# WeltXing/PyDyNet

Hardware: AMD Instinct MI355X
Metric: training-step samples/sec (6L Llama3, seq=256) (higher is better)
Workload: dtype f32

## Files before the change

pydynet_amd/csrc/common.h:

```cpp
#pragma once
#include <hip/hip_runtime.h>
#include <stdint.h>
#include <stdio.h>
#include <string.h>

#define PDN_MAX_DIMS 8

enum {
  PDN_OK = 0,
  PDN_EINVAL = -1,
  PDN_EUNSUPPORTED = -2,
  PDN_EWORKSPACE = -3,
};

void pdn_set_error(const char* fmt, ...);

enum {
  PDN_CNT_ROWRES_CHUNK = 0,
  PDN_CNT_ROWTILE_PLAIN = 1,
  PDN_CNT_ROWTILE_SWIGLU_FWD = 2,
  PDN_CNT_ROWTILE_SWIGLU_BWD = 3,
  PDN_CNT_ROWTILE_ROPE = 4,
  PDN_CNT_ROWTILE_ROWMAX = 5,
  PDN_CNT_ROWRES_CHUNK_EPI = 6,
  PDN_CNT_ATT_P_FWD = 7,
  PDN_CNT_ATT_P_BWD = 8,
  PDN_CNT_ATT_RES_FWD = 9,
  PDN_CNT_ATT_RES_BWD = 10,
  PDN_CNT_ATT_STREAM = 11,
  PDN_CNT_CE_DX_DEFERRED = 12,
  PDN_CNT_CE_DW = 13,
  PDN_CNT_OUTRES = 14,
  PDN_CNT_OUTRES_TN = 15,
  PDN_CNT_LINEAR_RELU_FWD = 16,
  PDN_CNT_LINEAR_DX_MASKED = 17,
  PDN_CNT_CE_SMALL = 18,
  PDN_CNT_TILED_SWIGLU_FWD = 19,
  PDN_CNT_TILED_SWIGLU_BWD = 20,
  PDN_CNT_CONV_QUAD_FWD = 21,
  PDN_CNT_CONV_QUAD_DGRAD = 22,
  PDN_CNT_CONV_QUAD_WGRAD = 23,
  PDN_CNT_PATCH_EMBED_FWD = 24,
  PDN_CNT_PATCH_EMBED_BWD = 25,
  PDN_CNT_L2NORM_FWD = 26,
  PDN_CNT_L2NORM_BWD = 27,
  PDN_CNT_SAMPLE = 28,
  PDN_CNT_DECODE_ROWS = 29,
  PDN_CNT_DECODE_SLOTS = 30,
  PDN_CNT_DECODE_WIDE = 31,
  PDN_CNT_BEAM = 32,
  PDN_CNT_EXTEND = 33,
  PDN_CNT_SPECULATE = 34,
  PDN_CNT_PENALTY = 35,
  PDN_CNT_LOGPROBS = 36,
  PDN_CNT_LMHEAD_SPLIT = 37,
  PDN_CNT_PREFIX = 38,
  PDN_CNT_CE_DX_SPLIT = 39,
  PDN_CNT_CE_DW_SPLIT = 40,
  PDN_CNT_ROWTILE_SPLIT = 41,
  PDN_CNT_OUTRES_TN_SPLIT = 42,
  PDN_CNT_ATT_SEG = 43,
  PDN_CNT_ROW_LOSS = 44,
  PDN_CNT_SMOOTH_LOSS = 45,
  PDN_CNT_OUTRES_SPLIT = 46,
  PDN_CNT_SLOTS = 47
};
void pdn_count(int slot);

#define PDN_CHECK_ARG(cond, ...)          \
  do {                                    \
    if (!(cond)) {                        \
      pdn_set_error(__VA_ARGS__);         \
      return PDN_EINVAL;                  \
    }                                     \
  } while (0)

#define PDN_LAUNCH_CHECK()                                            \
  do {                                                                \
    hipError_t _e = hipGetLastError();                                \
    if (_e != hipSuccess) {                                           \
      pdn_set_error("%s:%d launch failed: %s", __FILE__, __LINE__,    \
                    hipGetErrorString(_e));                           \
      return (int)_e;                                                 \
    }                                                                 \
  } while (0)

#define PDN_HIP(call)                                                 \
  do {                                                                \
    hipError_t _e = (call);                                           \
    if (_e != hipSuccess) {                                           \
      pdn_set_error("%s:%d %s: %s", __FILE__, __LINE__, #call,        \
                    hipGetErrorString(_e));                           \
      return (int)_e;                                                 \
    }                                                                 \
  } while (0)

static inline int64_t cdiv64(int64_t a, int64_t b) { return (a + b - 1) / b; }

struct PdnView {
  int ndim;
  int64_t shape[PDN_MAX_DIMS];
  int64_t stride[PDN_MAX_DIMS];
};

__device__ __forceinline__ float wave_sum(float v) {
#pragma unroll
  for (int o = 32; o > 0; o >>= 1) v += __shfl_xor(v, o, 64);
  return v;
}
__device__ __forceinline__ float wave_max(float v) {
#pragma unroll
  for (int o = 32; o > 0; o >>= 1) v = fmaxf(v, __shfl_xor(v, o, 64));
  return v;
}
__device__ __forceinline__ double wave_sum(double v) {
#pragma unroll
  for (int o = 32; o > 0; o >>= 1) v += __shfl_xor(v, o, 64);
  return v;
// ... 53 lines not shown
```

pydynet_amd/csrc/gemm.hip:

```cpp
#include "common.h"
#include <vector>
#include <mutex>
#include <stdlib.h>
#include <stdio.h>
#include <type_traits>

#include "gemm_tiled.h"
#include "gemm_stream.h"
#include "split_tn.h"

struct TileCfg {
  int waves_m, waves_n, wm, wn, bk;
  float eff;
};
static const TileCfg kCfgs[] = {
    {2, 2, 2, 2, 32, 1.00f},
    {4, 1, 1, 3, 32, 0.97f},
    {1, 4, 3, 1, 32, 0.95f},
    {4, 1, 1, 2, 32, 0.85f},
    {1, 4, 2, 1, 32, 0.90f},
    {2, 2, 1, 1, 32, 0.60f},
    {2, 2, 4, 2, 16, 0.85f},
    {2, 2, 2, 4, 16, 1.10f},
    {4, 1, 2, 3, 16, 0.99f},
// ... 72 lines not shown
#define PDN_GEMM_FAMILIES 5
extern "C" int pdn_gemm_prof_collect_families(double* ms5, double* flops5, int64_t* launches5) {
  std::lock_guard<std::mutex> lk(g_prof_mu);
  double ms[PDN_GEMM_FAMILIES] = {0}, fl[PDN_GEMM_FAMILIES] = {0};
  int64_t n[PDN_GEMM_FAMILIES] = {0};
  for (auto& r : g_prof) {
    PDN_HIP(hipEventSynchronize(r.e1));
    float t = 0.f;
    PDN_HIP(hipEventElapsedTime(&t, r.e0, r.e1));
    const int f = r.family == 5 ? 2 : (r.family < 0 || r.family >= PDN_GEMM_FAMILIES ? 0 : r.family);
    ms[f] += t; fl[f] += r.flops; n[f]++;
    (void)hipEventDestroy(r.e0);
    (void)hipEventDestroy(r.e1);
  }
  for (int f = 0; f < PDN_GEMM_FAMILIES; ++f) {
    if (ms5) ms5[f] = ms[f];
    if (flops5) flops5[f] = fl[f];
    if (launches5) launches5[f] = n[f];
  }
  g_prof.clear();
  return PDN_OK;
}

extern "C" int pdn_gemm_prof_collect(double* total_ms, double* total_flops, int64_t* launches) {
  double ms[PDN_GEMM_FAMILIES], fl[PDN_GEMM_FAMILIES];
  int64_t n[PDN_GEMM_FAMILIES];
  int rc = pdn_gemm_prof_collect_families(ms, fl, n);
  if (rc) return rc;
  double tm = 0, tf = 0;
  int64_t tn = 0;
  for (int f = 0; f < PDN_GEMM_FAMILIES; ++f) { tm += ms[f]; tf += fl[f]; tn += n[f]; }
  if (total_ms) *total_ms = tm;
  if (total_flops) *total_flops = tf;
  if (launches) *launches = tn;
  return PDN_OK;
}

int pdn_gemm_outres_tn_plan(int N, int K, int* nw_out, int* k_per_split_out);
int pdn_gemm_outres_tn_launch(const float* X, const float* G, float* C, int N, int K, int64_t ldx, int64_t ldg,
                              int64_t ldc, int64_t slab, int nw, int k_per_split, void* stream);
int pdn_gemm_outres_tn_blocks_launch(const float* X, const float* G, float* C, int N, int K, int64_t ldx, int64_t ldg,
                                     int nb_cols, int nw, int k_per_split, void* stream);
extern "C" int64_t pdn_gemm_outres_workspace_bytes(int M, int K);
extern "C" int pdn_gemm_outres_plan(int M, int K, int* nw, int* kps);
extern "C" int pdn_gemm_outres_ws_f32(const float* A, const float* B, float* C, const float* bias, const float* residual,
                                      int M, int N, int K, int64_t lda, int64_t ldb, int64_t ldc, int b_trans,
                                      void* workspace, int64_t workspace_bytes, void* stream);
extern "C" int pdn_gemm_outres_supported(int M, int N, int K, int64_t lda, int64_t ldb, int64_t ldc, int b_trans);
extern "C" int pdn_gemm_outres_f32(const float* A, const float* B, float* C, const float* bias,
                                   const float* residual, int M, int N, int K, int64_t lda, int64_t ldb,
                                   int64_t ldc, int b_trans, void* stream);
extern "C" int pdn_gemm_rowres_supported(int M, int N, int K, int64_t lda, int64_t ldb, int64_t ldc, int b_trans);
int pdn_rowtile_plain_ok(int M, int N, int b_trans);
extern "C" int pdn_gemm_rowres_f32(const float* A, const float* B, float* C, const float* bias,
                                   const float* residual, int M, int N, int K, int64_t lda, int64_t ldb,
                                   int64_t ldc, int b_trans, void* stream);
int pdn_gemm_rowres_blocks(const float* A, const float* B, float* C, int M, int N, int K, int64_t lda, int64_t ldb,
                           int64_t ldc, int b_trans, int nblocks, int64_t b_block_stride, void* stream);

extern "C" int64_t pdn_gemm_f32_workspace_bytes(int M, int N, int K, int nbatch) {
  const int64_t base = (int64_t)64 * M * N * (int64_t)nbatch * 4;
  if (!pdn_outres_tn_split_supported(M, N, nbatch, K)) return base;
  return ((base + 255) & ~(int64_t)255) + pdn_outres_tn_split_extra_bytes(K);
}

bool pdn_gemm_narrow_nn_ok(int M, int N, int K, int64_t a_rs, int64_t a_cs, const void* A);
int pdn_gemm_narrow_nn_launch(const float* A, int64_t lda, const float* B, int64_t b_rs, int64_t b_cs, const float* bias,
                              float* C, int64_t ldc, int M, int N, int K, void* stream);
int pdn_gemm_narrow_tn_plan(int Mc, int N, int K, int64_t a_rs, int64_t a_cs, int64_t b_cs, const void* A, int64_t ws_cap_floats,
                            int* kps);
int pdn_gemm_narrow_tn_launch(const float* A, int64_t a_cs, const float* B, int64_t b_rs, float* slabs, int Mc, int N, int K,
                              int kps, int splits, void* stream);

static int gemm_f32_impl(int M, int N, int K, float alpha, const float* A, int64_t a_rs,
                         int64_t a_cs, const float* B, int64_t b_rs, int64_t b_cs, float beta,
                         float* C, int64_t ldc, const float* bias, int nb1, int nb2,
                         int64_t a_bs1, int64_t a_bs2, int64_t b_bs1, int64_t b_bs2,
                         int64_t c_bs1, int64_t c_bs2, const float* residual,
                         float* b_colsum, int colsum_accumulate, void* workspace,
                         int64_t workspace_bytes, void* stream, uint32_t* relu_mask, const uint32_t* grad_mask,
                         float* mask_colsum = nullptr) {
  const bool ext_on = relu_mask || grad_mask;
  PDN_CHECK_ARG(!ext_on || (nb1 == 1 && nb2 == 1 && N % 32 == 0 && !b_colsum),
                "pdn_gemm_f32: the mask epilogues need one batch and N a multiple of 32 (N = %d)", N);
  PDN_CHECK_ARG(M >= 0 && N >= 0 && K >= 0 && nb1 >= 0 && nb2 >= 0, "pdn_gemm_f32: negative extent");
  if (M == 0 || N == 0 || nb1 == 0 || nb2 == 0) return PDN_OK;
  PDN_CHECK_ARG(A && B && C, "pdn_gemm_f32: null operand");
  PDN_CHECK_ARG(ldc >= N, "pdn_gemm_f32: ldc (%lld) < N (%d)", (long long)ldc, N);
  hipStream_t st = (hipStream_t)stream;
  const int nbatch = nb1 * nb2;

  GemmParams p;
  p.A = A; p.B = B; p.C = C; p.bias = bias; p.ws = (float*)workspace;
  p.residual = residual; p.colsum = b_colsum; p.colsum_acc = colsum_accumulate;
  p.relu_mask = relu_mask; p.grad_mask = grad_mask; p.mask_colsum = grad_mask ? mask_colsum : nullptr;
  p.M = M; p.N = N; p.K = K;
  p.a_rs = a_rs; p.a_cs = a_cs; p.b_rs = b_rs; p.b_cs = b_cs; p.ldc = ldc;
  p.nb2 = nb2;
  p.a_bs1 = a_bs1; p.a_bs2 = a_bs2; p.b_bs1 = b_bs1; p.b_bs2 = b_bs2; p.c_bs1 = c_bs1; p.c_bs2 = c_bs2;
  p.alpha = alpha; p.beta = beta;

  const bool a_kin = !(a_rs == 1 && a_cs != 1) || M == 1;
  const bool b_kin = (b_rs == 1 && b_cs != 1) || (b_rs == 1 && N == 1);
  auto al16 = [](const void* q) { return ((uintptr_t)q & 15) == 0; };
  auto m4 = [](int64_t v) { return (v & 3) == 0; };
  bool vec = al16(A) && al16(B) && m4(a_bs1) && m4(a_bs2) && m4(b_bs1) && m4(b_bs2);
// ... 26 lines not shown
      if (getenv("PDN_GEMM_DEBUG")) fprintf(stderr, "pdn_gemm_f32 M=%d N=%d K=%d -> narrow NN\n", M, N, K);
      return pdn_gemm_narrow_nn_launch(A, a_rs, B, b_rs, b_cs, bias, C, ldc, M, N, K, stream);
    }
    int kps = 0;
    const int64_t cap = (workspace && workspace_bytes > 0 && al16(workspace)) ? workspace_bytes / 4 : 0;
    const int sp = !bias ? pdn_gemm_narrow_tn_plan(M, N, K, a_rs, a_cs, b_cs, A, cap, &kps) : 0;
    if (sp > 0) {
      if (getenv("PDN_GEMM_DEBUG")) fprintf(stderr, "pdn_gemm_f32 M=%d N=%d K=%d -> narrow TN (%d slabs)\n", M, N, K, sp);
      const int rc = pdn_gemm_narrow_tn_launch(A, a_cs, B, b_rs, (float*)workspace, M, N, K, kps, sp, stream);
      if (rc) return rc;
      p.splits = sp;
      const int64_t total = (int64_t)M * N;
      const int blocks = (int)((total + 255) / 256 < 2048 ? (total + 255) / 256 : 2048);
      const int rvec = (N % 4 == 0) && (ldc % 4 == 0) && al16(C);
      hipLaunchKernelGGL(gemm_splitk_reduce_kernel, dim3(blocks), dim3(256), 0, st, p, 1, rvec);
      PDN_LAUNCH_CHECK();
      return PDN_OK;
    }
  }
  if (nbatch == 1 && !ext_on && N == 288 && a_cs == 1 && alpha == 1.f && beta == 0.f && !b_colsum && K >= 768 &&
      al16(A) && al16(B) && !getenv("PDN_GEMM_NO_OUTRES")) {
    const int bt = (b_rs == 1 && b_cs != 1) ? 1 : 0;
    const int64_t ldb = bt ? b_cs : b_rs;
    const bool big = (M + 255) / 256 >= 224, mid = (M + 127) / 128 >= 224 && K >= 1536;
    int pl_nw, pl_kps;
    const int64_t or_ws = (workspace && workspace_bytes > 0) ? workspace_bytes : 0;
    const bool cut = !big && M >= 8192 && K >= 1536 && pdn_gemm_outres_plan(M, K, &pl_nw, &pl_kps) > 1 &&
                     or_ws >= pdn_gemm_outres_workspace_bytes(M, K);
    if ((big || mid || cut) && (bt || b_cs == 1) && pdn_gemm_outres_supported(M, N, K, a_rs, ldb, ldc, bt)) {
      bool prof;
      ProfRec rec;
      {
        std::lock_guard<std::mutex> lk(g_prof_mu);
        prof = g_prof_on;
      }
      if (prof) {
        PDN_HIP(hipEventCreate(&rec.e0));
        PDN_HIP(hipEventCreate(&rec.e1));
        rec.flops = 2.0 * M * (double)N * (double)K;
        rec.family = 3;
        PDN_HIP(hipEventRecord(rec.e0, st));
      }
      if (getenv("PDN_GEMM_DEBUG"))
        fprintf(stderr, "pdn_gemm_f32 M=%d N=%d K=%d -> output-resident (%s)\n", M, N, K, bt ? "NT" : "NN");
      const int rc = cut ? pdn_gemm_outres_ws_f32(A, B, C, bias, residual, M, N, K, a_rs, ldb, ldc, bt, workspace, or_ws, stream)
                         : pdn_gemm_outres_f32(A, B, C, bias, residual, M, N, K, a_rs, ldb, ldc, bt, stream);
      if (rc) return rc;
      if (prof) {
        PDN_HIP(hipEventRecord(rec.e1, st));
        std::lock_guard<std::mutex> lk(g_prof_mu);
        g_prof.push_back(rec);
      }
      return PDN_OK;
    }
  }
  {
    const bool one_dim = nb1 == 1 || nb2 == 1;
    const int64_t a_bs = nb1 == 1 ? a_bs2 : a_bs1, b_bs = nb1 == 1 ? b_bs2 : b_bs1, c_bs = nb1 == 1 ? c_bs2 : c_bs1;
    const bool blocks = nbatch > 1 && one_dim && a_bs == 0 && c_bs == N && ldc >= (int64_t)nbatch * N && !bias &&
                        N % 96 == 0 && (b_bs & 3) == 0;
    const int64_t n_all = (int64_t)N * (blocks ? nbatch : 1);
    const int bt0 = (b_rs == 1 && b_cs != 1) ? 1 : 0;
    const bool tilepiece = nbatch == 1 && K == 288 && n_all >= 96 && n_all % 32 == 0 && M >= 8192 &&
                           pdn_rowtile_plain_ok(M, (int)n_all, bt0);
    if ((nbatch == 1 || blocks) && !ext_on && K == 288 && a_cs == 1 && alpha == 1.f && beta == 0.f && !b_colsum &&
        (tilepiece || (!residual && n_all >= 768)) && n_all < (1 << 30) && M >= 8192 && al16(A) && al16(B) &&
        (!residual || al16(residual)) && !getenv("PDN_GEMM_NO_ROWRES")) {
      const int bt = (b_rs == 1 && b_cs != 1) ? 1 : 0;
      const int64_t ldb = bt ? b_cs : b_rs;
      if ((bt || b_cs == 1) && pdn_gemm_rowres_supported(M, N, K, a_rs, ldb, ldc, bt)) {
        bool prof;
        ProfRec rec;
        {
          std::lock_guard<std::mutex> lk(g_prof_mu);
          prof = g_prof_on;
        }
        if (prof) {
          PDN_HIP(hipEventCreate(&rec.e0));
          PDN_HIP(hipEventCreate(&rec.e1));
          rec.flops = 2.0 * M * (double)n_all * (double)K;
          rec.family = 2;
          PDN_HIP(hipEventRecord(rec.e0, st));
        }
        if (getenv("PDN_GEMM_DEBUG"))
          fprintf(stderr, "pdn_gemm_f32 M=%d N=%lld K=%d -> row-resident (%s, %d block%s)\n", M, (long long)n_all, K,
                  bt ? "NT" : "NN", blocks ? nbatch : 1, blocks ? "s" : "");
        const int rc = blocks ? pdn_gemm_rowres_blocks(A, B, C, M, (int)n_all, K, a_rs, ldb, ldc, bt, nbatch, b_bs, stream)
                              : pdn_gemm_rowres_f32(A, B, C, bias, residual, M, N, K, a_rs, ldb, ldc, bt, stream);
        if (rc) return rc;
        if (prof) {
          PDN_HIP(hipEventRecord(rec.e1, st));
          std::lock_guard<std::mutex> lk(g_prof_mu);
          g_prof.push_back(rec);
        }
        return PDN_OK;
      }
    }
  }
  const int64_t ws_cap = (workspace && workspace_bytes > 0) ? workspace_bytes / 4 : 0;
  if (nbatch == 1 && !ext_on && M == 288 && a_rs == 1 && a_cs >= 288 && b_cs == 1 && alpha == 1.f && !b_colsum && !bias && !residual &&
      N >= 8192 && N % 32 == 0 && K % 32 == 0 && K >= 4096 && m4(a_cs) && m4(b_rs) && al16(A) && al16(B) &&
      (int64_t)288 * ldc < (1ll << 30) && (int64_t)32 * b_rs < (1ll << 30) && !getenv("PDN_GEMM_NO_OUTRES")) {
    int nw = 8, kps = K;
    const int splits = pdn_gemm_outres_tn_plan(N, K, &nw, &kps);
    const bool direct = splits == 1 && beta == 0.f;
    if (direct || (int64_t)splits * M * N <= ws_cap) {
// ... 562 lines not shown
```

pydynet_amd/csrc/gemm_outres.hip:

```cpp
#include "common.h"
#include <stdlib.h>

static int pdn_ablation_switch(const char* name) {
  const char* e = getenv(name);
  const int v = e ? atoi(e) : 0;
  if (v) fprintf(stderr, "[pdnhip] WARNING: %s=%d -- timing ablation active, results of the affected kernels are WRONG\n", name, v);
  return v;
}

typedef float f32x16 __attribute__((ext_vector_type(16)));

struct OutResParams {
  const float* A;
  const float* B;
  float* C;
  const float* bias;
  const float* residual;
  int M, K;
  int64_t lda, ldb, ldc;
  const float* lse;
  const int64_t* targets;
  const float* gdev;
  float gscale;
  int kps;
// ... 346 lines not shown
  int nw, kps;
  const int splits = pdn_gemm_outres_plan(M, K, &nw, &kps);
  return splits > 1 ? (int64_t)splits * M * OR_N * 4 : 0;
}

extern "C" int pdn_gemm_outres_supported(int M, int N, int K, int64_t lda, int64_t ldb, int64_t ldc, int b_trans) {
  return N == OR_N && K >= OR_KP && K % OR_KP == 0 && M >= 1 && lda % 4 == 0 && ldb % 4 == 0 && lda >= K &&
         ldb >= (b_trans ? K : N) && ldc >= N && (int64_t)OR_N * ldb < (1ll << 30) && (int64_t)32 * ldc < (1ll << 30);
}

static int outres_launch(const float* A, const float* B, float* C, const float* bias, const float* residual, int M, int N,
                         int K, int64_t lda, int64_t ldb, int64_t ldc, int b_trans, void* workspace,
                         int64_t workspace_bytes, void* stream, int kb = 0, int64_t b_bstride = 0);

extern "C" int pdn_gemm_outres_f32(const float* A, const float* B, float* C, const float* bias,
                                   const float* residual, int M, int N, int K, int64_t lda, int64_t ldb,
                                   int64_t ldc, int b_trans, void* stream) {
  return outres_launch(A, B, C, bias, residual, M, N, K, lda, ldb, ldc, b_trans, nullptr, 0, stream);
}

extern "C" int pdn_gemm_outres_ws_f32(const float* A, const float* B, float* C, const float* bias,
                                      const float* residual, int M, int N, int K, int64_t lda, int64_t ldb,
                                      int64_t ldc, int b_trans, void* workspace, int64_t workspace_bytes, void* stream) {
  return outres_launch(A, B, C, bias, residual, M, N, K, lda, ldb, ldc, b_trans, workspace, workspace_bytes, stream);
}

int pdn_gemm_prof_begin(int family, double flops, double bytes, void* stream);
void pdn_gemm_prof_end(int token, void* stream);

extern "C" int pdn_gemm_outres_blocks_supported(int M, int kb, int nb) {
  const int K = kb * nb;
  const bool big = (M + 255) / 256 >= 224, mid = (M + 127) / 128 >= 224 && K >= 1536;
  return (kb > 0 && kb % OR_KP == 0 && nb >= 1 && (big || mid)) ? 1 : 0;
}
extern "C" int pdn_gemm_outres_blocks_nt_f32(const float* A, const float* W, int64_t b_block_stride, int kb, int nb, float* C,
                                             const float* residual, int M, int64_t lda, int64_t ldc, void* stream) {
  if (M == 0) return PDN_OK;
  const int K = kb * nb;
  if (!pdn_gemm_outres_blocks_supported(M, kb, nb) || (b_block_stride & 3) || (kb & 3) ||
      !pdn_gemm_outres_supported(M, OR_N, K, lda, K, ldc, 1)) {
    pdn_set_error("pdn_gemm_outres_blocks_nt_f32: unsupported shape M=%d kb=%d nb=%d", M, kb, nb);
    return PDN_EUNSUPPORTED;
  }
  const int tk = pdn_gemm_prof_begin(3, 2.0 * M * (double)OR_N * K, 0.0, stream);
  const int rc = outres_launch(A, W, C, nullptr, residual, M, OR_N, K, lda, kb, ldc, 1, nullptr, 0, stream, kb, b_block_stride);
  pdn_gemm_prof_end(tk, stream);
  return rc;
}

int pdn_outres_split_takes(const float* A, const float* B, const float* C, const float* bias, const float* residual, int M,
                           int K, int64_t lda, int64_t ldb, int64_t ldc, int b_trans, int kb, int64_t b_bstride, int splits,
                           void* stream);
int pdn_outres_split_launch(const float* A, const float* B, float* C, const float* bias, const float* residual, int M, int K,
                            int64_t lda, int64_t ldb, int64_t ldc, int b_trans, int kb, int64_t b_bstride, void* stream);

static int outres_launch(const float* A, const float* B, float* C, const float* bias, const float* residual, int M, int N,
                         int K, int64_t lda, int64_t ldb, int64_t ldc, int b_trans, void* workspace,
                         int64_t workspace_bytes, void* stream, int kb, int64_t b_bstride) {
  if (M == 0 || N == 0) return PDN_OK;
  PDN_CHECK_ARG(A && B && C, "pdn_gemm_outres_f32: null operand");
  if (!pdn_gemm_outres_supported(M, N, K, lda, kb > 0 ? K : ldb, ldc, b_trans)) {
    pdn_set_error("pdn_gemm_outres_f32: unsupported shape M=%d N=%d K=%d (N 288, K a multiple of 32, leading "
                  "dimensions multiples of 4)", M, N, K);
    return PDN_EUNSUPPORTED;
  }
  PDN_CHECK_ARG(((((uintptr_t)A | (uintptr_t)B) & 15) == 0), "pdn_gemm_outres_f32: 16-byte alignment required");
  OutResParams p{A, B, C, bias, residual, M, K, lda, ldb, ldc, nullptr, nullptr, nullptr, 0.f, K / OR_KP, nullptr};
  static const int s_pdn_outres_rt_ablate = pdn_ablation_switch("PDN_OUTRES_RT_ABLATE");
  p.ablate_rt = s_pdn_outres_rt_ablate;
  if (kb > 0) {
    p.ppb = kb / OR_KP;
    p.ppb_magic = (unsigned)(((1ull << 32) + (unsigned)p.ppb - 1) / (unsigned)p.ppb);
    p.b_bstride = b_bstride;
  }
  hipStream_t st = (hipStream_t)stream;
  int plan_nw = 8, kps = K / OR_KP;
  int splits = pdn_gemm_outres_plan(M, K, &plan_nw, &kps);
  if (splits > 1 && (!workspace || workspace_bytes < (int64_t)splits * M * OR_N * 4 || (ldc & 3) ||
                     ((uintptr_t)C & 15) || ((uintptr_t)workspace & 15) || ((uintptr_t)bias & 15) || ((uintptr_t)residual & 15))) {
    splits = 1;
    plan_nw = outres_unsplit_nw(M);
  }
  if (splits > 1) { p.kps = kps; p.slab = (float*)workspace; }
  if (pdn_outres_split_takes(A, B, C, bias, residual, M, K, lda, ldb, ldc, b_trans, kb, b_bstride, splits, stream)) {
    const int rc = pdn_outres_split_launch(A, B, C, bias, residual, M, K, lda, ldb, ldc, b_trans, kb, b_bstride, stream);
    if (rc == PDN_OK) pdn_count(PDN_CNT_OUTRES);
    return rc;
  }
  static const int nw_env = getenv("PDN_OUTRES_NW") ? atoi(getenv("PDN_OUTRES_NW")) : 0;
  static const int stage_env = getenv("PDN_OUTRES_STAGE") ? atoi(getenv("PDN_OUTRES_STAGE")) : -1;
  static const int ablate = pdn_ablation_switch("PDN_OUTRES_ABLATE");
  const int nw = nw_env ? nw_env : plan_nw;
  const int stage = stage_env >= 0 ? stage_env : 1;
  const dim3 grid((M + 32 * nw - 1) / (32 * nw), splits);
  pdn_count(PDN_CNT_OUTRES);
#define OR_LAUNCH(BT_, NW_, ST_, AB_) hipLaunchKernelGGL((gemm_outres_kernel<BT_, NW_, ST_, AB_>), grid, dim3(NW_ * 64), 0, st, p)
  if (ablate == 1 && b_trans) OR_LAUNCH(true, 4, 1, 1);
  else if (ablate == 2 && b_trans) OR_LAUNCH(true, 4, 1, 2);
  else if (nw == 8 && b_trans) { if (stage) OR_LAUNCH(true, 8, 1, 0); else OR_LAUNCH(true, 8, 0, 0); }
  else if (nw == 8) { if (stage) OR_LAUNCH(false, 8, 1, 0); else OR_LAUNCH(false, 8, 0, 0); }
  else if (b_trans) { if (stage) OR_LAUNCH(true, 4, 1, 0); else OR_LAUNCH(true, 4, 0, 0); }
  else { if (stage) OR_LAUNCH(false, 4, 1, 0); else OR_LAUNCH(false, 4, 0, 0); }
#undef OR_LAUNCH
  PDN_LAUNCH_CHECK();
  if (splits > 1) {
    const int64_t n4 = (int64_t)M * (OR_N / 4);
    hipLaunchKernelGGL(outres_splitk_reduce_kernel, dim3((unsigned)((n4 + 255) / 256)), dim3(256), 0, st, p.slab, splits, M,
                       bias, residual, C, ldc);
    PDN_LAUNCH_CHECK();
  }
  return PDN_OK;
}

int pdn_outres_ce_dx_launch(const float* logits, int64_t ldl, const float* lse, const int64_t* targets, float gscale,
                            const float* gdev, const float* W, int64_t ldw, float* dx, int64_t ldc,
                            const float* residual, int M, int V, void* workspace, int64_t workspace_bytes, void* stream) {
  OutResParams p{logits, W, dx, nullptr, residual, M, V, ldl, ldw, ldc, lse, targets, gdev, gscale, V / OR_KP, nullptr};
  int nw = 8, kps = V / OR_KP;
  int splits = pdn_gemm_outres_plan(M, V, &nw, &kps);
  if (splits > 1 && (!workspace || workspace_bytes < (int64_t)splits * M * OR_N * 4 || (ldc & 3) || ((uintptr_t)dx & 15) ||
                     ((uintptr_t)workspace & 15) || ((uintptr_t)residual & 15))) {
    splits = 1;
    nw = outres_unsplit_nw(M);
  }
  if (splits > 1) { p.kps = kps; p.slab = (float*)workspace; }
  const dim3 grid((M + 32 * nw - 1) / (32 * nw), splits);
  if (nw == 8) hipLaunchKernelGGL((gemm_outres_kernel<true, 8, 1, 0, 1>), grid, dim3(512), 0, (hipStream_t)stream, p);
  else hipLaunchKernelGGL((gemm_outres_kernel<true, 4, 1, 0, 1>), grid, dim3(256), 0, (hipStream_t)stream, p);
  PDN_LAUNCH_CHECK();
  if (splits > 1) {
    const int64_t n4 = (int64_t)M * (OR_N / 4);
    hipLaunchKernelGGL(outres_splitk_reduce_kernel, dim3((unsigned)((n4 + 255) / 256)), dim3(256), 0, (hipStream_t)stream,
                       p.slab, splits, M, (const float*)nullptr, residual, dx, ldc);
    PDN_LAUNCH_CHECK();
  }
  return PDN_OK;
}

// ... 409 lines not shown
```

pydynet_amd/csrc/outres_split.hip:

```cpp
#include "split_tn.h"
#include "outres_split_index.h"

extern "C" int pdn_malloc(void** ptr, int64_t bytes);
extern "C" int pdn_free(void* ptr);

struct OrsWParams {
  const float* B;
  float* pmax;
  int* wsh;
  char* wimg;
  int np, ppb;
  int64_t ldb, bstride;
};

__device__ __forceinline__ float ors_finite_or_inf(float a) { return a < INFINITY ? a : INFINITY; }

template <bool NN>
__device__ __forceinline__ void ors_w_unit(const OrsWParams& p, const float* tile, int d, int q, float (&v)[8]) {
  if (NN) {
#pragma unroll
    for (int j = 0; j < 8; ++j) v[j] = tile[ors_nn_lds(8 * q + j, d)];
  } else {
    const float* src = p.B + ors_w_src_nt(blockIdx.x, d, q, p.ppb, p.ldb, p.bstride);
    const float4 a = *reinterpret_cast<const float4*>(src);
    const float4 b = *reinterpret_cast<const float4*>(src + 4);
    v[0] = a.x; v[1] = a.y; v[2] = a.z; v[3] = a.w; v[4] = b.x; v[5] = b.y; v[6] = b.z; v[7] = b.w;
  }
}
__device__ __forceinline__ void ors_w_stage_nn(const OrsWParams& p, float* tile) {
  for (int i = threadIdx.x; i < ORS_KP * (ORS_N / 4); i += 256) {
    const float4 a = *reinterpret_cast<const float4*>(p.B + ors_w_src_nn(blockIdx.x, i, p.ldb));
    float* t = tile + ors_nn_lds(i / 72, 4 * (i % 72));
    t[0] = a.x; t[1] = a.y; t[2] = a.z; t[3] = a.w;
  }
  __syncthreads();
}

template <bool NN>
__global__ __launch_bounds__(256) void ors_w_max_kernel(OrsWParams p) {
  __shared__ float tile[NN ? ORS_KP * ORS_NN_LD : 1];
  if (NN) ors_w_stage_nn(p, tile);
  for (int i = threadIdx.x; i < ORS_N * 4; i += 256) {
    const int d = i >> 2, q = i & 3;
    float v[8];
    ors_w_unit<NN>(p, tile, d, q, v);
    float m = 0.f;
#pragma unroll
    for (int j = 0; j < 8; ++j) m = fmaxf(m, ors_finite_or_inf(fabsf(v[j])));
    m = fmaxf(m, __shfl_xor(m, 1, 64));
    m = fmaxf(m, __shfl_xor(m, 2, 64));
    if (q == 0) p.pmax[(int64_t)blockIdx.x * ORS_N + d] = m;
  }
}

template <bool NN>
__global__ __launch_bounds__(256) void ors_w_img_kernel(OrsWParams p) {
  __shared__ float tile[NN ? ORS_KP * ORS_NN_LD : 1];
  if (NN) ors_w_stage_nn(p, tile);
  char* img = p.wimg + (int64_t)blockIdx.x * ORS_PIECE;
  for (int i = threadIdx.x; i < ORS_N * 4; i += 256) {
    const int d = i >> 2, q = i & 3;
    float amax = 0.f;
    for (int s = 0; s < p.np; ++s) amax = fmaxf(amax, p.pmax[(int64_t)s * ORS_N + d]);
    const int sh = ls_shift(amax);
    if (blockIdx.x == 0 && q == 0) p.wsh[d] = sh;
    float v[8];
    ors_w_unit<NN>(p, tile, d, q, v);
    f16x8 hv, lv;
#pragma unroll
    for (int j = 0; j < 8; ++j) {
      _Float16 h, l;
      ls_split(v[j], sh, h, l);
      hv[j] = h; lv[j] = l;
    }
    char* dst = img + ors_img_unit(d, q);
    *reinterpret_cast<f16x8*>(dst) = hv;
    *reinterpret_cast<f16x8*>(dst + ORS_PLANE) = lv;
  }
}

struct OrsParams {
  const float* A;
  const char* wimg;
  const int* wsh;
  const float* bias;
  const float* residual;
  float* C;
  int M, np, nblk;
  int64_t lda, ldc;
};

__device__ __forceinline__ float ors_max8(const float4& a, const float4& b) {
  const float v[8] = {a.x, a.y, a.z, a.w, b.x, b.y, b.z, b.w};
  float m = 0.f;
#pragma unroll
  for (int j = 0; j < 8; ++j) {
    const float f = fabsf(v[j]);
    m = fmaxf(m, f < INFINITY ? f : 0.f);
  }
  return m;
}
__device__ __forceinline__ int ors_step_exp(float mx, int S) { return ors_next_exp(mx > 0.f, __builtin_amdgcn_frexp_expf(mx), S); }
__device__ __forceinline__ void ors_form2(float x0, float x1, int S, unsigned& hp, unsigned& lp) {
  f16x2 h, l;
  _Float16 a, b;
  ls_split_scaled(ldexpf(x0, S), a, b);
  h[0] = a; l[0] = b;
  ls_split_scaled(ldexpf(x1, S), a, b);
  h[1] = a; l[1] = b;
  hp = __builtin_bit_cast(unsigned, h);
  lp = __builtin_bit_cast(unsigned, l);
  asm volatile("" : "+v"(hp), "+v"(lp));
}

template <int ABLATE>
__global__ __launch_bounds__(512, 1) void ors_main_kernel(OrsParams p) {
  __shared__ __attribute__((aligned(1024))) char smem[ORS_LDS];
  const int tid = threadIdx.x, lane = tid & 63;
  const int wave = __builtin_amdgcn_readfirstlane(tid >> 6);
  const int r = lane & 15, q = lane >> 4;
  const int np = p.np, nblk = p.nblk, grid = gridDim.x;
  const unsigned lds0 = (unsigned)(size_t)(__attribute__((address_space(3))) char*)smem;
  constexpr bool STREAM = ABLATE == 0 || ABLATE == 3;

  const char* wsrc = p.wimg + lane * 16;
  auto dma_w = [&](int piece, int slot) __attribute__((always_inline)) {
    const char* src = wsrc + (int64_t)piece * ORS_PIECE;
#pragma unroll
    for (int e = 0; e < 5; ++e) {
      const int I = ors_wdma_instr(e, wave);
      split_dma16(src + I * 1024, __builtin_amdgcn_readfirstlane(lds0 + slot + I * 1024));
    }
  };
  auto a_src = [&](int blk, int i) __attribute__((always_inline)) {
    return p.A + ors_a_row(blk, wave, ors_raw_row(i, lane), p.M) * p.lda + 4 * ors_raw_chunk(i, lane);
  };
  int blk = blockIdx.x, nxt = ors_next_block(blk, grid, nblk);
  const float* ac0 = a_src(blk, 0);
  const float* ac1 = a_src(blk, 1);
  const float* an0 = a_src(nxt, 0);
  const float* an1 = a_src(nxt, 1);
  const int rw_base = ORS_RING0 + wave * (ORS_RING * ORS_RAW);
  auto dma_raw = [&](const float* s0, const float* s1, int piece, int ring) __attribute__((always_inline)) {
    const int64_t o = (int64_t)piece * ORS_KP;
    split_dma16(s0 + o, __builtin_amdgcn_readfirstlane(lds0 + rw_base + ring * ORS_RAW));
    split_dma16(s1 + o, __builtin_amdgcn_readfirstlane(lds0 + rw_base + ring * ORS_RAW + 1024));
  };
  const int raw_lane = rw_base + ors_raw_lane(r, q);

  dma_w(0, 0);
  if (ABLATE != 1) { dma_raw(ac0, ac1, 0, 0); dma_raw(ac0, ac1, 1, 1); dma_raw(ac0, ac1, 2, 2); dma_raw(ac0, ac1, 3, 3); }
  asm volatile("s_waitcnt vmcnt(0)" ::: "memory");
  f16x8 bh, bl;
#pragma unroll
  for (int j = 0; j < 8; ++j) { bh[j] = (_Float16)1.f; bl[j] = (_Float16)0.5f; }
  int S = ABLATE == 1 ? 0 : ORS_UNSET;
  if (ABLATE != 1) {
    const float4 v0 = *reinterpret_cast<const float4*>(__builtin_assume_aligned(smem + raw_lane, 16));
    const float4 v1 = *reinterpret_cast<const float4*>(__builtin_assume_aligned(smem + (raw_lane ^ 16), 16));
    float mx = ors_max8(v0, v1);
    mx = fmaxf(mx, __shfl_xor(mx, 16, 64));
    mx = fmaxf(mx, __shfl_xor(mx, 32, 64));
    S = ors_step_exp(mx, S);
    unsigned h0, h1, h2, h3, l0, l1, l2, l3;
    ors_form2(v0.x, v0.y, S, h0, l0);
    ors_form2(v0.z, v0.w, S, h1, l1);
    ors_form2(v1.x, v1.y, S, h2, l2);
    ors_form2(v1.z, v1.w, S, h3, l3);
    bh = stn_pack4(h0, h1, h2, h3); bl = stn_pack4(l0, l1, l2, l3);
  }

  f32x4 acc0[ORS_NT], acc1[ORS_NT];
#pragma unroll
  for (int j = 0; j < ORS_NT; ++j)
#pragma unroll
    for (int i = 0; i < 4; ++i) { acc0[j][i] = 0.f; acc1[j][i] = 0.f; }
// ... 28 lines not shown
          dma_w(last ? 0 : s + 1, ORS_PIECE - cur);
          if (STREAM) {
            const bool ahead = ors_ahead_next(s, np);
            dma_raw(ahead ? an0 : ac0, ahead ? an1 : ac1, ors_ahead_piece(s, np), g & (ORS_RING - 1));
          }
          if (ABLATE != 1) {
            const int ro = raw_lane + ((g + 1) & (ORS_RING - 1)) * ORS_RAW;
            rv0 = *reinterpret_cast<const float4*>(__builtin_assume_aligned(smem + ro, 16));
            rv1 = *reinterpret_cast<const float4*>(__builtin_assume_aligned(smem + (ro ^ 16), 16));
          }
        }
        __builtin_amdgcn_sched_barrier(0);
        acc0[j] = __builtin_amdgcn_mfma_f32_16x16x32_f16(wh[j & 1], bh, acc0[j], 0, 0, 0);
        acc1[j] = __builtin_amdgcn_mfma_f32_16x16x32_f16(wl[j & 1], bh, acc1[j], 0, 0, 0);
        acc1[j] = __builtin_amdgcn_mfma_f32_16x16x32_f16(wh[j & 1], bl, acc1[j], 0, 0, 0);
        if (ABLATE != 1) {
          if (j == 1) { mx = ors_max8(rv0, rv1); mo = __shfl_xor(mx, 16, 64); }
          if (j == 2) { mx = fmaxf(mx, mo); mo = __shfl_xor(mx, 32, 64); }
          if (j == 3) { mx = fmaxf(mx, mo); Sn = ors_step_exp(mx, Sn); }
          if (j >= 5 && (j - 5) % 3 == 0 && j <= 14) {
            const int e = (j - 5) / 3;
            const float4 rv = (e >> 1) ? rv1 : rv0;
            unsigned hp, lp;
            ors_form2((e & 1) ? rv.z : rv.x, (e & 1) ? rv.w : rv.y, Sn, hp, lp);
            if (e == 0) { nh.x = hp; nl.x = lp; } else if (e == 1) { nh.y = hp; nl.y = lp; }
            else if (e == 2) { nh.z = hp; nl.z = lp; } else { nh.w = hp; nl.w = lp; }
            __builtin_amdgcn_sched_group_barrier(0x008, 1, 0);
            __builtin_amdgcn_sched_group_barrier(0x002, 6, 0);
            __builtin_amdgcn_sched_group_barrier(0x008, 1, 0);
            __builtin_amdgcn_sched_group_barrier(0x002, 6, 0);
            __builtin_amdgcn_sched_group_barrier(0x008, 1, 0);
          }
        }
        __builtin_amdgcn_sched_barrier(0);
      }
#undef ORS_LOADW
      bh = __builtin_bit_cast(f16x8, nh); bl = __builtin_bit_cast(f16x8, nl);
      cur = ORS_PIECE - cur;
      if (last) {
        Snext = Sn;
      } else {
        if (__builtin_amdgcn_ballot_w64(Sn != S) != 0) {
          const float f = ldexpf(1.f, Sn - S);
#pragma unroll
          for (int j = 0; j < ORS_NT; ++j) { acc0[j] *= f; acc1[j] *= f; }
        }
        S = Sn;
      }
    }

    const int64_t row = (int64_t)blk * ORS_WG_ROWS + wave * 16 + r;
    if ((ABLATE != 3 || p.M < 0) && row < p.M) {
      float* out = p.C + row * p.ldc + 4 * q;
      const float* res = p.residual ? p.residual + row * p.ldc + 4 * q : nullptr;
      const float* bia = p.bias ? p.bias + 4 * q : nullptr;
      const int* __restrict__ shp = p.wsh + 4 * q;
#pragma unroll
      for (int j = 0; j < ORS_NT; ++j) {
        const int4 sv = *reinterpret_cast<const int4*>(shp + 16 * j);
        float4 o;
        o.x = stn_unscale(acc1[j][0], acc0[j][0], S + sv.x);
        o.y = stn_unscale(acc1[j][1], acc0[j][1], S + sv.y);
        o.z = stn_unscale(acc1[j][2], acc0[j][2], S + sv.z);
        o.w = stn_unscale(acc1[j][3], acc0[j][3], S + sv.w);
        if (bia) { const float4 b4 = *reinterpret_cast<const float4*>(bia + 16 * j); o.x += b4.x; o.y += b4.y; o.z += b4.z; o.w += b4.w; }
        if (res) { const float4 r4 = *reinterpret_cast<const float4*>(res + 16 * j); o.x += r4.x; o.y += r4.y; o.z += r4.z; o.w += r4.w; }
        *reinterpret_cast<float4*>(out + 16 * j) = o;
      }
    }
    asm volatile("s_waitcnt vmcnt(0)" ::: "memory");
    if (nxt == blk) break;
    blk = nxt;
    nxt = ors_next_block(blk, grid, nblk);
    ac0 = an0; ac1 = an1;
    an0 = a_src(nxt, 0); an1 = a_src(nxt, 1);
    S = ABLATE == 1 ? 0 : Snext;
#pragma unroll
    for (int j = 0; j < ORS_NT; ++j)
#pragma unroll
      for (int i = 0; i < 4; ++i) { acc0[j][i] = 0.f; acc1[j][i] = 0.f; }
  }
}

namespace {
struct OrsTemp {
  void* p = nullptr;
  hipStream_t st = nullptr;
  int get(int64_t bytes, void* stream) { st = (hipStream_t)stream; return pdn_malloc(&p, bytes); }
  ~OrsTemp() {
    static const bool two_stream = getenv("PDN_TWO_STREAM") && atoi(getenv("PDN_TWO_STREAM")) != 0;
    if (p && two_stream) (void)hipStreamSynchronize(st);
    if (p) pdn_free(p);
  }
};
}

int pdn_outres_split_takes(const float* A, const float* B, const float* C, const float* bias, const float* residual, int M,
                           int K, int64_t lda, int64_t ldb, int64_t ldc, int b_trans, int kb, int64_t b_bstride, int splits,
                           void* stream) {
  if (M < ORS_MIN_ROWS || K < ORS_MIN_K || K > ORS_MAX_K || K % ORS_KP != 0 || splits != 1) return 0;
  if ((lda & 3) || (ldc & 3) || (ldb & 3) || (b_bstride & 3) || lda < K || ldc < ORS_N) return 0;
  if (kb > 0 ? (!b_trans || kb % ORS_KP != 0 || K % kb != 0) : ldb < (b_trans ? K : ORS_N)) return 0;
  if (((uintptr_t)A | (uintptr_t)B | (uintptr_t)C | (uintptr_t)bias | (uintptr_t)residual) & 15) return 0;
  const char* e = getenv("PDN_OUTRES_SPLIT");
  if (e && atoi(e) == 0) {
    static bool s_told = false;
    if (!s_told) {
      s_told = true;
      fprintf(stderr, "[pdnhip] WARNING: PDN_OUTRES_SPLIT=0 -- the layer input gradients and the down projection stay on the fp32 MFMA kernel\n");
    }
    return 0;
  }
  hipStreamCaptureStatus cs = hipStreamCaptureStatusNone;
  if (hipStreamIsCapturing((hipStream_t)stream, &cs) != hipSuccess) { (void)hipGetLastError(); return 0; }
  return cs == hipStreamCaptureStatusNone ? 1 : 0;
}

int pdn_outres_split_launch(const float* A, const float* B, float* C, const float* bias, const float* residual, int M, int K,
                            int64_t lda, int64_t ldb, int64_t ldc, int b_trans, int kb, int64_t b_bstride, void* stream) {
  const char* ea = getenv("PDN_OUTRES_SPLIT_ABLATE");
  const int ablate = ea ? atoi(ea) : 0;
  if (ablate != 0) {
    static bool s_told = false;
    if (!s_told) {
      s_told = true;
      fprintf(stderr, "[pdnhip] WARNING: PDN_OUTRES_SPLIT_ABLATE=%d -- timing ablation active, the results of the split output-resident products are WRONG\n", ablate);
    }
  }
  const char* eg = getenv("PDN_OUTRES_SPLIT_WGS");
  const int env_wgs = eg ? atoi(eg) : -1;
  const int np = K / ORS_KP;
  OrsTemp tmp;
  const int rc = tmp.get((int64_t)np * ORS_PIECE + (int64_t)np * ORS_N * 4 + ORS_N * 4, stream);
  if (rc) return rc;
  hipStream_t st = (hipStream_t)stream;
  OrsWParams w;
  memset(&w, 0, sizeof(w));
  w.B = B; w.wimg = static_cast<char*>(tmp.p); w.pmax = reinterpret_cast<float*>(w.wimg + (int64_t)np * ORS_PIECE);
  w.wsh = reinterpret_cast<int*>(w.pmax + (int64_t)np * ORS_N);
  w.np = np; w.ppb = kb > 0 ? kb / ORS_KP : np; w.ldb = ldb; w.bstride = kb > 0 ? b_bstride : 0;
  if (b_trans) {
    hipLaunchKernelGGL(ors_w_max_kernel<false>, dim3(np), dim3(256), 0, st, w);
    hipLaunchKernelGGL(ors_w_img_kernel<false>, dim3(np), dim3(256), 0, st, w);
  } else {
    hipLaunchKernelGGL(ors_w_max_kernel<true>, dim3(np), dim3(256), 0, st, w);
    hipLaunchKernelGGL(ors_w_img_kernel<true>, dim3(np), dim3(256), 0, st, w);
  }
  OrsParams p;
  memset(&p, 0, sizeof(p));
  p.A = A; p.wimg = w.wimg; p.wsh = w.wsh; p.bias = bias; p.residual = residual; p.C = C;
  p.M = M; p.np = np; p.nblk = ors_blocks(M); p.lda = lda; p.ldc = ldc;
  int wgs = ors_grid(M);
  if (env_wgs == 0) wgs = p.nblk;
  else if (env_wgs > 0) wgs = ors_min_i(env_wgs, p.nblk);
  const dim3 grid((unsigned)wgs);
  if (ablate == 3) hipLaunchKernelGGL(ors_main_kernel<3>, grid, dim3(512), 0, st, p);
  else STN_LAUNCH_ABLATE(ors_main_kernel, ablate, grid, stream, p);
  pdn_count(PDN_CNT_OUTRES_SPLIT);
  PDN_LAUNCH_CHECK();
  return PDN_OK;
}
```

pydynet_amd/csrc/outres_split_index.h:

```cpp
#pragma once
#include <stdint.h>

#if defined(__HIPCC__) || defined(__CUDACC__)
#define ORS_HD __host__ __device__ __forceinline__
#else
#define ORS_HD inline
#endif

#define ORS_N 288
#define ORS_NT 18
#define ORS_KP 32
#define ORS_PLANE (ORS_N * ORS_KP * 2)
#define ORS_PIECE (2 * ORS_PLANE)
#define ORS_RAW 2048
#define ORS_RING 4
#define ORS_WG_ROWS 128
#define ORS_RING0 (2 * ORS_PIECE)
#define ORS_LDS (ORS_RING0 + 8 * ORS_RING * ORS_RAW)
#define ORS_MAX_WGS 256
#define ORS_MIN_ROWS 65536
#define ORS_MIN_K 256
#define ORS_MAX_K 4096
#define ORS_NN_LD 289

ORS_HD int ors_min_i(int a, int b) { return a < b ? a : b; }
ORS_HD int64_t ors_min_l(int64_t a, int64_t b) { return a < b ? a : b; }

ORS_HD int ors_blocks(int64_t M) { return (int)((M + ORS_WG_ROWS - 1) / ORS_WG_ROWS); }
ORS_HD int ors_grid(int64_t M) { return ors_min_i(ors_blocks(M), ORS_MAX_WGS); }
ORS_HD int ors_next_block(int blk, int grid, int nblk) { return blk + grid < nblk ? blk + grid : blk; }

ORS_HD int ors_img_unit(int d, int q) { return (d * 4 + (q ^ ((d >> 2) & 3))) * 16; }
ORS_HD int ors_frag(int r, int q) { return ors_img_unit(r, q); }
ORS_HD int64_t ors_w_src_nt(int piece, int d, int q, int ppb, int64_t ldb, int64_t bstride) {
  const int b = piece / ppb;
  return (int64_t)b * bstride + (int64_t)d * ldb + (int64_t)(piece - b * ppb) * ORS_KP + 8 * q;
}
ORS_HD int64_t ors_w_src_nn(int piece, int i, int64_t ldb) { return ((int64_t)piece * ORS_KP + i / 72) * ldb + 4 * (i % 72); }
ORS_HD int ors_nn_lds(int k, int d) { return k * ORS_NN_LD + d; }
ORS_HD int ors_wdma_instr(int e, int wave) { return ors_min_i(e * 8 + wave, 35); }

ORS_HD int ors_raw_row(int i, int lane) { return 8 * i + (lane >> 3); }
ORS_HD int ors_raw_chunk(int i, int lane) { return (lane & 7) ^ ((ors_raw_row(i, lane) >> 1) & 7); }
ORS_HD int64_t ors_a_row(int blk, int wave, int rr, int64_t M) { return ors_min_l((int64_t)blk * ORS_WG_ROWS + wave * 16 + rr, M - 1); }
ORS_HD int ors_raw_lane(int r, int q) { return r * 128 + (((2 * q) ^ ((r >> 1) & 7)) << 4); }
ORS_HD int ors_ahead_piece(int s, int np) { return s + ORS_RING < np ? s + ORS_RING : s + ORS_RING - np; }
ORS_HD bool ors_ahead_next(int s, int np) { return s + ORS_RING >= np; }

ORS_HD int ors_out_col(int j, int q) { return 16 * j + 4 * q; }

#define ORS_UNSET (1 << 20)
ORS_HD int ors_next_exp(bool nonzero, int E, int S) { return (nonzero && E + S >= 16) ? 13 - E : S; }
```

Baseline: 8463.

## Route 288x288 projection GEMMs to the split-fp16 output-resident kernel

Adds a dispatch path in the generic GEMM entry so that single-batch N=K=288 products (attention projections) use the split-fp16 output-resident kernel when it accepts the shape. The weight image kernel now spreads over a 2D grid instead of looping per block. Per-column shifts and bias are staged in LDS, and residual loads in the epilogue are double-buffered in groups. Risks include the precision behaviour of the split fp16 path on more layers and added LDS use in the main kernel.

New measurement: 8662 (median of 6 runs). 2.3% higher.

```diff
diff --git a/pydynet_amd/csrc/common.h b/pydynet_amd/csrc/common.h
--- a/pydynet_amd/csrc/common.h
+++ b/pydynet_amd/csrc/common.h
@@ -63,7 +63,8 @@
   PDN_CNT_ROW_LOSS = 44,
   PDN_CNT_SMOOTH_LOSS = 45,
   PDN_CNT_OUTRES_SPLIT = 46,
-  PDN_CNT_SLOTS = 47
+  PDN_CNT_PROJ288_SPLIT = 47,
+  PDN_CNT_SLOTS = 48
 };
 void pdn_count(int slot);
 
diff --git a/pydynet_amd/csrc/gemm.hip b/pydynet_amd/csrc/gemm.hip
--- a/pydynet_amd/csrc/gemm.hip
+++ b/pydynet_amd/csrc/gemm.hip
@@ -148,6 +148,13 @@
                                    int64_t ldc, int b_trans, void* stream);
 extern "C" int pdn_gemm_rowres_supported(int M, int N, int K, int64_t lda, int64_t ldb, int64_t ldc, int b_trans);
 int pdn_rowtile_plain_ok(int M, int N, int b_trans);
+extern "C" int pdn_gemm_rowtile_mode(int mode);
+int pdn_outres_split_takes(const float* A, const float* B, const float* C, const float* bias, const float* residual, int M,
+                           int K, int64_t lda, int64_t ldb, int64_t ldc, int b_trans, int kb, int64_t b_bstride, int splits,
+                           void* stream);
+int pdn_outres_split_launch(const float* A, const float* B, float* C, const float* bias, const float* residual, int M, int K,
+                            int64_t lda, int64_t ldb, int64_t ldc, int b_trans, int kb, int64_t b_bstride, void* stream,
+                            int count_slot);
 extern "C" int pdn_gemm_rowres_f32(const float* A, const float* B, float* C, const float* bias,
                                    const float* residual, int M, int N, int K, int64_t lda, int64_t ldb,
                                    int64_t ldc, int b_trans, void* stream);
@@ -280,6 +287,25 @@
         g_prof.push_back(rec);
       }
       return PDN_OK;
+    }
+  }
+  if (nbatch == 1 && !ext_on && N == 288 && K == 288 && a_cs == 1 && alpha == 1.f && beta == 0.f && !b_colsum &&
+      !getenv("PDN_GEMM_NO_OUTRES") && !getenv("PDN_GEMM_NO_ROWRES") && pdn_gemm_rowtile_mode(-1) != 3) {
+    const int bt = (b_rs == 1 && b_cs != 1) ? 1 : 0;
+    const int64_t ldb = bt ? b_cs : b_rs;
+    auto overlaps_c = [&](const float* q, int64_t floats) {
+      return q && q < (const float*)C + (int64_t)M * ldc && (const float*)C < q + floats;
+    };
+    if ((bt || b_cs == 1) && pdn_rowtile_plain_ok(M, N, bt) && pdn_gemm_rowres_supported(M, N, K, a_rs, ldb, ldc, bt) &&
+        !overlaps_c(A, (int64_t)M * a_rs) && !overlaps_c(B, (int64_t)288 * ldb) &&
+        (residual == C || !overlaps_c(residual, (int64_t)M * ldc)) &&
+        pdn_outres_split_takes(A, B, C, bias, residual, M, K, a_rs, ldb, ldc, bt, 0, 0, 1, stream)) {
+      if (getenv("PDN_GEMM_DEBUG"))
+        fprintf(stderr, "pdn_gemm_f32 M=%d N=%d K=%d -> output-resident, split fp16 (%s)\n", M, N, K, bt ? "NT" : "NN");
+      const int tk = pdn_gemm_prof_begin(3, 2.0 * M * (double)N * (double)K, 0.0, stream);
+      const int rc = pdn_outres_split_launch(A, B, C, bias, residual, M, K, a_rs, ldb, ldc, bt, 0, 0, stream, PDN_CNT_PROJ288_SPLIT);
+      pdn_gemm_prof_end(tk, stream);
+      return rc;
     }
   }
   {
diff --git a/pydynet_amd/csrc/gemm_outres.hip b/pydynet_amd/csrc/gemm_outres.hip
--- a/pydynet_amd/csrc/gemm_outres.hip
+++ b/pydynet_amd/csrc/gemm_outres.hip
@@ -422,7 +422,8 @@
                            int K, int64_t lda, int64_t ldb, int64_t ldc, int b_trans, int kb, int64_t b_bstride, int splits,
                            void* stream);
 int pdn_outres_split_launch(const float* A, const float* B, float* C, const float* bias, const float* residual, int M, int K,
-                            int64_t lda, int64_t ldb, int64_t ldc, int b_trans, int kb, int64_t b_bstride, void* stream);
+                            int64_t lda, int64_t ldb, int64_t ldc, int b_trans, int kb, int64_t b_bstride, void* stream,
+                            int count_slot);
 
 static int outres_launch(const float* A, const float* B, float* C, const float* bias, const float* residual, int M, int N,
                          int K, int64_t lda, int64_t ldb, int64_t ldc, int b_trans, void* workspace,
@@ -453,7 +454,8 @@
   }
   if (splits > 1) { p.kps = kps; p.slab = (float*)workspace; }
   if (pdn_outres_split_takes(A, B, C, bias, residual, M, K, lda, ldb, ldc, b_trans, kb, b_bstride, splits, stream)) {
-    const int rc = pdn_outres_split_launch(A, B, C, bias, residual, M, K, lda, ldb, ldc, b_trans, kb, b_bstride, stream);
+    const int rc = pdn_outres_split_launch(A, B, C, bias, residual, M, K, lda, ldb, ldc, b_trans, kb, b_bstride, stream,
+                                           PDN_CNT_OUTRES_SPLIT);
     if (rc == PDN_OK) pdn_count(PDN_CNT_OUTRES);
     return rc;
   }
diff --git a/pydynet_amd/csrc/outres_split.hip b/pydynet_amd/csrc/outres_split.hip
--- a/pydynet_amd/csrc/outres_split.hip
+++ b/pydynet_amd/csrc/outres_split.hip
@@ -58,7 +58,8 @@
   __shared__ float tile[NN ? ORS_KP * ORS_NN_LD : 1];
   if (NN) ors_w_stage_nn(p, tile);
   char* img = p.wimg + (int64_t)blockIdx.x * ORS_PIECE;
-  for (int i = threadIdx.x; i < ORS_N * 4; i += 256) {
+  const int i = blockIdx.y * 256 + threadIdx.x;
+  if (i < ORS_N * 4) {
     const int d = i >> 2, q = i & 3;
     float amax = 0.f;
     for (int s = 0; s < p.np; ++s) amax = fmaxf(amax, p.pmax[(int64_t)s * ORS_N + d]);
@@ -122,6 +123,10 @@
   const int np = p.np, nblk = p.nblk, grid = gridDim.x;
   const unsigned lds0 = (unsigned)(size_t)(__attribute__((address_space(3))) char*)smem;
   constexpr bool STREAM = ABLATE == 0 || ABLATE == 3;
+  __shared__ __attribute__((aligned(16))) int col_sh[ORS_N];
+  __shared__ __attribute__((aligned(16))) float col_bias[ORS_N];
+  if (tid < ORS_N) { col_sh[tid] = p.wsh[tid]; col_bias[tid] = p.bias ? p.bias[tid] : -0.f; }
+  asm volatile("s_waitcnt vmcnt(0) lgkmcnt(0)" ::: "memory");
 
   const char* wsrc = p.wimg + lane * 16;
   auto dma_w = [&](int piece, int slot) __attribute__((always_inline)) {
@@ -256,20 +261,39 @@
     const int64_t row = (int64_t)blk * ORS_WG_ROWS + wave * 16 + r;
     if ((ABLATE != 3 || p.M < 0) && row < p.M) {
       float* out = p.C + row * p.ldc + 4 * q;
-      const float* res = p.residual ? p.residual + row * p.ldc + 4 * q : nullptr;
-      const float* bia = p.bias ? p.bias + 4 * q : nullptr;
-      const int* __restrict__ shp = p.wsh + 4 * q;
-#pragma unroll
-      for (int j = 0; j < ORS_NT; ++j) {
-        const int4 sv = *reinterpret_cast<const int4*>(shp + 16 * j);
+      auto tile_out = [&](int j) __attribute__((always_inline)) {
+        const int4 sv = *reinterpret_cast<const int4*>(__builtin_assume_aligned(col_sh + 16 * j + 4 * q, 16));
+        const float4 b4 = *reinterpret_cast<const float4*>(__builtin_assume_aligned(col_bias + 16 * j + 4 * q, 16));
         float4 o;
-        o.x = stn_unscale(acc1[j][0], acc0[j][0], S + sv.x);
-        o.y = stn_unscale(acc1[j][1], acc0[j][1], S + sv.y);
-        o.z = stn_unscale(acc1[j][2], acc0[j][2], S + sv.z);
-        o.w = stn_unscale(acc1[j][3], acc0[j][3], S + sv.w);
-        if (bia) { const float4 b4 = *reinterpret_cast<const float4*>(bia + 16 * j); o.x += b4.x; o.y += b4.y; o.z += b4.z; o.w += b4.w; }
-        if (res) { const float4 r4 = *reinterpret_cast<const float4*>(res + 16 * j); o.x += r4.x; o.y += r4.y; o.z += r4.z; o.w += r4.w; }
-        *reinterpret_cast<float4*>(out + 16 * j) = o;
+        o.x = stn_unscale(acc1[j][0], acc0[j][0], S + sv.x) + b4.x;
+        o.y = stn_unscale(acc1[j][1], acc0[j][1], S + sv.y) + b4.y;
+        o.z = stn_unscale(acc1[j][2], acc0[j][2], S + sv.z) + b4.z;
+        o.w = stn_unscale(acc1[j][3], acc0[j][3], S + sv.w) + b4.w;
+        return o;
+      };
+      if (p.residual) {
+        const float* res = p.residual + row * p.ldc + 4 * q;
+        float4 rq[2][ORS_DRAIN];
+#pragma unroll
+        for (int i = 0; i < ORS_DRAIN; ++i) rq[0][i] = *reinterpret_cast<const float4*>(res + 16 * i);
+#pragma unroll
+        for (int g = 0; g < ORS_NT / ORS_DRAIN; ++g) {
+          if (g + 1 < ORS_NT / ORS_DRAIN) {
+#pragma unroll
+            for (int i = 0; i < ORS_DRAIN; ++i) rq[(g + 1) & 1][i] = *reinterpret_cast<const float4*>(res + 16 * ((g + 1) * ORS_DRAIN + i));
+          }
+#pragma unroll
+          for (int i = 0; i < ORS_DRAIN; ++i) {
+            const int j = g * ORS_DRAIN + i;
+            float4 o = tile_out(j);
+            const float4 r4 = rq[g & 1][i];
+            o.x += r4.x; o.y += r4.y; o.z += r4.z; o.w += r4.w;
+            *reinterpret_cast<float4*>(out + 16 * j) = o;
+          }
+        }
+      } else {
+#pragma unroll
+        for (int j = 0; j < ORS_NT; ++j) *reinterpret_cast<float4*>(out + 16 * j) = tile_out(j);
       }
     }
     asm volatile("s_waitcnt vmcnt(0)" ::: "memory");
@@ -311,7 +335,7 @@
     static bool s_told = false;
     if (!s_told) {
       s_told = true;
-      fprintf(stderr, "[pdnhip] WARNING: PDN_OUTRES_SPLIT=0 -- the layer input gradients and the down projection stay on the fp32 MFMA kernel\n");
+      fprintf(stderr, "[pdnhip] WARNING: PDN_OUTRES_SPLIT=0 -- the layer input gradients, the down projection and the 288 x 288 products stay on the fp32 MFMA kernels\n");
     }
     return 0;
   }
@@ -321,7 +345,8 @@
 }
 
 int pdn_outres_split_launch(const float* A, const float* B, float* C, const float* bias, const float* residual, int M, int K,
-                            int64_t lda, int64_t ldb, int64_t ldc, int b_trans, int kb, int64_t b_bstride, void* stream) {
+                            int64_t lda, int64_t ldb, int64_t ldc, int b_trans, int kb, int64_t b_bstride, void* stream,
+                            int count_slot) {
   const char* ea = getenv("PDN_OUTRES_SPLIT_ABLATE");
   const int ablate = ea ? atoi(ea) : 0;
   if (ablate != 0) {
@@ -345,10 +370,10 @@
   w.np = np; w.ppb = kb > 0 ? kb / ORS_KP : np; w.ldb = ldb; w.bstride = kb > 0 ? b_bstride : 0;
   if (b_trans) {
     hipLaunchKernelGGL(ors_w_max_kernel<false>, dim3(np), dim3(256), 0, st, w);
-    hipLaunchKernelGGL(ors_w_img_kernel<false>, dim3(np), dim3(256), 0, st, w);
+    hipLaunchKernelGGL(ors_w_img_kernel<false>, dim3(np, ORS_IMG_WGS), dim3(256), 0, st, w);
   } else {
     hipLaunchKernelGGL(ors_w_max_kernel<true>, dim3(np), dim3(256), 0, st, w);
-    hipLaunchKernelGGL(ors_w_img_kernel<true>, dim3(np), dim3(256), 0, st, w);
+    hipLaunchKernelGGL(ors_w_img_kernel<true>, dim3(np, ORS_IMG_WGS), dim3(256), 0, st, w);
   }
   OrsParams p;
   memset(&p, 0, sizeof(p));
@@ -360,7 +385,7 @@
   const dim3 grid((unsigned)wgs);
   if (ablate == 3) hipLaunchKernelGGL(ors_main_kernel<3>, grid, dim3(512), 0, st, p);
   else STN_LAUNCH_ABLATE(ors_main_kernel, ablate, grid, stream, p);
-  pdn_count(PDN_CNT_OUTRES_SPLIT);
+  pdn_count(count_slot);
   PDN_LAUNCH_CHECK();
   return PDN_OK;
 }
diff --git a/pydynet_amd/csrc/outres_split_index.h b/pydynet_amd/csrc/outres_split_index.h
--- a/pydynet_amd/csrc/outres_split_index.h
+++ b/pydynet_amd/csrc/outres_split_index.h
@@ -17,6 +17,8 @@
 #define ORS_WG_ROWS 128
 #define ORS_RING0 (2 * ORS_PIECE)
 #define ORS_LDS (ORS_RING0 + 8 * ORS_RING * ORS_RAW)
+#define ORS_IMG_WGS ((ORS_N * 4 + 255) / 256)
+#define ORS_DRAIN 6
 #define ORS_MAX_WGS 256
 #define ORS_MIN_ROWS 65536
 #define ORS_MIN_K 256
```
